# tyt0223/emqx

Measured on AMD Instinct MI355X. Metric: topics matched/sec (node) at 10M filters, 1/2/4/8 GPUs; % HBM roofline, higher is better.
Workload: dtype u32

## Files before the change

### emqx_amd/csrc/egm_bulk.cpp

```cpp
#include <stdio.h>
#include <stdlib.h>
#include <string.h>

#include <chrono>

#include <algorithm>
#include <string_view>
#include <thread>
#include <unordered_map>
#include <vector>

#include "egm_table.h"

namespace egm {

namespace {

template <class F>
void parallel_for(size_t n, unsigned nt, F fn) {
  if (n < nt) nt = (unsigned)n;
  if (nt <= 1) {
    fn((size_t)0, n, 0u);
    return;
  }
  std::vector<std::thread> th;
  for (unsigned t = 0; t < nt; ++t) {
    const size_t lo = n * t / nt, hi = n * (t + 1) / nt;
    th.emplace_back([=, &fn] { fn(lo, hi, t); });
  }
  for (auto& x : th) x.join();
}

template <class T>
void parallel_sort(std::vector<T>& v, unsigned nt) {
  const size_t n = v.size();
  if (nt <= 1 || n < (1u << 16)) {
    std::sort(v.begin(), v.end());
    return;
  }
  std::vector<size_t> b(nt + 1);
  for (unsigned t = 0; t <= nt; ++t) b[t] = n * t / nt;
  parallel_for(nt, nt, [&](size_t lo, size_t hi, unsigned) {
    for (size_t t = lo; t < hi; ++t) std::sort(v.begin() + b[t], v.begin() + b[t + 1]);
  });
  std::vector<T> tmp(n);
  std::vector<T>* src = &v;
  std::vector<T>* dst = &tmp;
  for (size_t w = 1; w < nt; w <<= 1) {
    std::vector<std::thread> th;
    for (size_t t = 0; t < nt; t += 2 * w) {
      const size_t a = b[t], m = b[std::min<size_t>(t + w, nt)], e = b[std::min<size_t>(t + 2 * w, nt)];
      th.emplace_back([=] { std::merge(src->begin() + a, src->begin() + m, src->begin() + m, src->begin() + e,
                                       dst->begin() + a); });
    }
    for (auto& x : th) x.join();
    std::swap(src, dst);
  }
  if (src != &v) v.swap(*src);
}

struct Item {
  uint64_t key;
  uint32_t li;
  uint32_t pad;
  bool operator<(const Item& o) const { return key != o.key ? key < o.key : li < o.li; }
};

template <class K>
std::vector<std::vector<uint32_t>> bin_by_range(size_t n, unsigned R, unsigned nt, K key) {
  std::vector<std::vector<std::vector<uint32_t>>> part(nt, std::vector<std::vector<uint32_t>>(R));
  parallel_for(n, nt, [&](size_t lo, size_t hi, unsigned t) {
    for (size_t i = lo; i < hi; ++i) {
      const uint32_t r = key(i);
      if (r < R) part[t][r].push_back((uint32_t)i);
    }
  });
  std::vector<std::vector<uint32_t>> out(R);
  parallel_for(R, nt, [&](size_t lo, size_t hi, unsigned) {
    for (size_t r = lo; r < hi; ++r)
      for (unsigned t = 0; t < nt; ++t) {
        out[r].insert(out[r].end(), part[t][r].begin(), part[t][r].end());
        std::vector<uint32_t>().swap(part[t][r]);
      }
  });
  return out;
}


}

unsigned build_threads() {
  const char* e = getenv("EGM_BUILD_THREADS");
  if (e && *e) return (unsigned)std::max(1, atoi(e));
  unsigned n = std::max(1u, std::thread::hardware_concurrency());
  if (FILE* f = fopen("/sys/fs/cgroup/cpu.max", "r")) {
    char q[64] = {0};
    unsigned long long period = 0;
    if (fscanf(f, "%63s %llu", q, &period) == 2 && strcmp(q, "max") != 0 && period) {
      const unsigned long long quota = strtoull(q, nullptr, 10);
      n = std::min<unsigned>(n, (unsigned)std::max<unsigned long long>(1, (quota + period - 1) / period));
    }
    fclose(f);
  }
  return std::min(n, 64u);
}

namespace {
struct Phase {
  bool on = getenv("EGM_BULK_TRACE") != nullptr;
  std::chrono::steady_clock::time_point t = std::chrono::steady_clock::now();
  void operator()(const char* what) {
    if (!on) return;
    const auto now = std::chrono::steady_clock::now();
    fprintf(stderr, "[egm bulk] %-22s %8.3f s\n", what, std::chrono::duration<double>(now - t).count());
    t = now;
  }
};
}

int HostTable::bulk_build(const uint8_t* blob, const uint32_t* off, uint32_t n, const uint32_t* ids, unsigned nt) {
  Phase phase;
  clear();
  if (nt == 0) nt = build_threads();
  std::vector<uint64_t> h(n);
  parallel_for(n, nt, [&](size_t lo, size_t hi, unsigned) {
    for (size_t i = lo; i < hi; ++i) h[i] = word_hash(blob + off[i], off[i + 1] - off[i]);
  });
  std::vector<uint8_t> dup(n, 0);
  {
    std::vector<Item> byh(n);
    parallel_for(n, nt, [&](size_t lo, size_t hi, unsigned) {
      for (size_t i = lo; i < hi; ++i) byh[i] = Item{h[i], (uint32_t)i, 0};
    });
    parallel_sort(byh, nt);
    parallel_for(n, nt, [&](size_t lo, size_t hi, unsigned) {
      for (size_t k = lo; k < hi; ++k) {
        if (k == 0 || byh[k - 1].key != byh[k].key) continue;
        const uint32_t i = byh[k].li, li = off[i + 1] - off[i];
        for (size_t j = k; j-- > 0 && byh[j].key == byh[k].key;) {
          const uint32_t p = byh[j].li;
          if (off[p + 1] - off[p] == li && memcmp(blob + off[p], blob + off[i], li) == 0) {
            dup[i] = 1;
            break;
          }
        }
      }
    });
  }
  phase("dedup");
  std::vector<uint32_t> uniq;
  uniq.reserve(n);
  for (uint32_t i = 0; i < n; ++i)
    if (!dup[i]) uniq.push_back(i);
  std::vector<uint8_t>().swap(dup);
  const uint32_t U = (uint32_t)uniq.size();
  foff_.assign((size_t)U + 1, 0);
  for (uint32_t r = 0; r < U; ++r) foff_[r + 1] = foff_[r] + (off[uniq[r] + 1] - off[uniq[r]]);
  fblob_.resize(foff_[U]);
  ffid_.resize(U);
  falive_.assign(U, 1);
  uint32_t max_fid = 0;
  parallel_for(U, nt, [&](size_t lo, size_t hi, unsigned) {
    for (size_t r = lo; r < hi; ++r) {
      const uint32_t i = uniq[r];
      memcpy(fblob_.data() + foff_[r], blob + off[i], off[i + 1] - off[i]);
      ffid_[r] = ids ? ids[i] : i;
    }
  });
  for (uint32_t r = 0; r < U; ++r) max_fid = std::max(max_fid, ffid_[r] + 1);
  n_filters_ = U;
  next_fid_ = U ? max_fid : 0;
  {
    std::vector<uint64_t> hb(U), hf(U);
    parallel_for(U, nt, [&](size_t lo, size_t hi, unsigned) {
      for (size_t r = lo; r < hi; ++r) {
        hb[r] = h[uniq[r]];
        hf[r] = mix64(ffid_[r]);
      }
    });
    std::vector<uint64_t>().swap(h);
    by_bytes_.bulk_build(hb, nt);
    by_fid_.bulk_build(hf, nt);
  }
  phase("filter store + maps");
  std::vector<uint64_t> tok_off((size_t)U + 1, 0);
  {
    std::vector<uint32_t> depth(U);
    parallel_for(U, nt, [&](size_t lo, size_t hi, unsigned) {
      for (size_t r = lo; r < hi; ++r) {
        const uint8_t* p = fblob_.data() + foff_[r];
        const uint64_t len = foff_[r + 1] - foff_[r];
        uint32_t d = 1;
        for (uint64_t k = 0; k < len; ++k) d += p[k] == '/';
        depth[r] = d;
      }
    });
    for (uint32_t r = 0; r < U; ++r) tok_off[r + 1] = tok_off[r] + depth[r];
  }
  std::vector<uint32_t> tok(tok_off[U]);
  {
    const unsigned T = (U < 4096) ? 1u : nt;
    std::vector<std::vector<std::string_view>> local(T);
    std::vector<std::vector<uint32_t>> to_global(T);
    parallel_for(U, T, [&](size_t lo, size_t hi, unsigned t) {
      std::unordered_map<std::string_view, uint32_t> seen;
      auto& lw = local[t];
      for (size_t r = lo; r < hi; ++r) {
        const uint8_t* p = fblob_.data() + foff_[r];
        const uint32_t len = (uint32_t)(foff_[r + 1] - foff_[r]);
        uint64_t o = tok_off[r];
        uint32_t s = 0;
        for (uint32_t i = 0; i <= len; ++i) {
          if (i < len && p[i] != '/') continue;
          const uint32_t wl = i - s;
          uint32_t v;
          if (wl == 1 && p[s] == '+') v = WID_PLUS;
          else if (wl == 1 && p[s] == '#') v = WID_HASH;
          else {
            std::string_view w((const char*)p + s, wl);
            auto it = seen.find(w);
            if (it == seen.end()) {
              it = seen.emplace(w, (uint32_t)lw.size()).first;
              lw.push_back(w);
            }
            v = it->second;
          }
          tok[o++] = v;
          s = i + 1;
        }
      }
    });
    size_t total = 0;
    for (auto& l : local) total += l.size();
    size_t cap = 64;
    while (cap < 2 * total) cap <<= 1;
    dict_rehash(cap);
    for (unsigned t = 0; t < T; ++t) {
      to_global[t].resize(local[t].size());
      for (size_t k = 0; k < local[t].size(); ++k)
        to_global[t][k] = dict_add((const uint8_t*)local[t][k].data(), (uint32_t)local[t][k].size());
    }
    parallel_for(U, T, [&](size_t lo, size_t hi, unsigned t) {
      const auto& g = to_global[t];
      for (uint64_t k = tok_off[lo]; k < tok_off[hi]; ++k)
        if (tok[k] < WID_MAX) tok[k] = g[tok[k]];
    });
  }
  phase("dictionary + tokens");
  std::vector<uint32_t> act(U), nxt;
  for (uint32_t r = 0; r < U; ++r) act[r] = r;
  std::vector<uint32_t> cur_node(U, 0);
  std::vector<NodeRec> nn(1, NodeRec{NONE, NONE, NONE, 0});
  std::vector<uint32_t> npar(1, NONE), nvia(1, NONE), nref(1, U), nhc(1, NONE);
  {
    const size_t bound = (size_t)tok_off[U] + 1;
    nn.reserve(bound + bound / 8 + 1024);
    for (auto* v : {&npar, &nvia, &nref, &nhc}) v->reserve(bound + bound / 8 + 1024);
  }
  struct Child {
    uint32_t token, first, count, start;
  };
  for (uint32_t level = 0; !act.empty(); ++level) {
    const size_t A = act.size();
    std::vector<size_t> cb{0};
    for (unsigned t = 1; t < nt; ++t) {
      size_t k = std::max(cb.back(), A * t / nt);
      while (k < A && k > 0 && cur_node[act[k]] == cur_node[act[k - 1]]) ++k;
      if (k > cb.back() && k < A) cb.push_back(k);
    }
    cb.push_back(A);
    const size_t C = cb.size() - 1;
    std::vector<std::vector<std::pair<uint64_t, uint32_t>>> citems(C);
    std::vector<std::vector<Child>> ckids(C);
    auto sort_chunk = [&](size_t c, unsigned inner) {
      auto& it = citems[c];
      auto& kids = ckids[c];
      it.resize(cb[c + 1] - cb[c]);
      for (size_t k = cb[c]; k < cb[c + 1]; ++k) {
        const uint32_t r = act[k];
        it[k - cb[c]] = {((uint64_t)tok[tok_off[r] + level] << 32) | r, cur_node[r]};
      }
      size_t a = 0;
      while (a < it.size()) {
        size_t e = a + 1;
        while (e < it.size() && it[e].second == it[a].second) ++e;
        if (e - a > 1) {
          if (inner > 1) {
            std::vector<std::pair<uint64_t, uint32_t>> run(it.begin() + a, it.begin() + e);
            parallel_sort(run, inner);
            std::copy(run.begin(), run.end(), it.begin() + a);
          } else {
            std::sort(it.begin() + a, it.begin() + e);
          }
        }
        const size_t k0 = kids.size();
        for (size_t k = a; k < e; ++k)
          if (k == a || (it[k].first >> 32) != (it[k - 1].first >> 32))
            kids.push_back(Child{(uint32_t)(it[k].first >> 32), (uint32_t)it[k].first, 0, (uint32_t)k});
        for (size_t g = k0; g < kids.size(); ++g)
          kids[g].count = (uint32_t)((g + 1 < kids.size() ? kids[g + 1].start : e) - kids[g].start);
        std::sort(kids.begin() + k0, kids.end(), [](const Child& x, const Child& y) { return x.first < y.first; });
        a = e;
      }
    };
    if (C == 1) sort_chunk(0, nt);
    else parallel_for(C, (unsigned)C, [&](size_t lo, size_t hi, unsigned) {
      for (size_t c = lo; c < hi; ++c) sort_chunk(c, 1);
    });
    std::vector<uint64_t> cbase(C + 1, nn.size());
    for (size_t c = 0; c < C; ++c) cbase[c + 1] = cbase[c] + ckids[c].size();
    if (cbase[C] >= (uint64_t)WID_MAX) return -1;
    const uint32_t N2 = (uint32_t)cbase[C];
    nn.resize(N2, NodeRec{NONE, NONE, NONE, 0});
    npar.resize(N2);
    nvia.resize(N2);
    nref.resize(N2);
    nhc.resize(N2, NONE);
    std::vector<uint64_t> nbase(C + 1, 0);
    std::vector<std::vector<uint32_t>> cnext(C);
    parallel_for(C, (unsigned)std::min<size_t>(C, nt), [&](size_t lo, size_t hi, unsigned) {
      for (size_t c = lo; c < hi; ++c) {
        const auto& it = citems[c];
        auto& out = cnext[c];
        out.reserve(it.size());
        for (size_t g = 0; g < ckids[c].size(); ++g) {
          const Child& k = ckids[c][g];
          const uint32_t node = (uint32_t)(cbase[c] + g), p = it[k.start].second;
          npar[node] = p;
          nvia[node] = k.token;
          nref[node] = k.count;
          if (k.token == WID_PLUS) nn[p].plus_child = node;
          else if (k.token == WID_HASH) nhc[p] = node;
          for (size_t q = k.start; q < (size_t)k.start + k.count; ++q) {
            const uint32_t r = (uint32_t)it[q].first;
            cur_node[r] = node;
            if (tok_off[r] + level + 1 == tok_off[r + 1]) {
              nn[node].term_fid = ffid_[r];
              if (k.token == WID_HASH) nn[p].hash_fid = ffid_[r];
            } else {
              out.push_back(r);
            }
          }
        }
        std::vector<std::pair<uint64_t, uint32_t>>().swap(citems[c]);
      }
    });
    for (size_t c = 0; c < C; ++c) nbase[c + 1] = nbase[c] + cnext[c].size();
    nxt.resize(nbase[C]);
    parallel_for(C, (unsigned)std::min<size_t>(C, nt), [&](size_t lo, size_t hi, unsigned) {
      for (size_t c = lo; c < hi; ++c) std::copy(cnext[c].begin(), cnext[c].end(), nxt.begin() + nbase[c]);
    });
    act.swap(nxt);
    phase("  level");
  }
  std::vector<uint32_t>().swap(cur_node);
  std::vector<uint32_t>().swap(tok);
  const uint32_t N = (uint32_t)nn.size();
  nodes.swap(nn);
  hash_child.swap(nhc);
  parent_.swap(npar);
  via_.swap(nvia);
  ref_.swap(nref);
  lit_count_.assign(N, 0);
  sig_.assign(N, 0);
  edge_slot_.assign(N, NONE);
  free_nodes_.clear();
  n_live_nodes_ = N;
  uint64_t n_lit = 0;
  for (uint32_t c = 1; c < N; ++c)
    if (via_[c] < WID_MAX) {
      ++lit_count_[parent_[c]];
      sig_[parent_[c]] |= sig_bit(via_[c]);
      ++n_lit;
    }
  parallel_for(N, nt, [&](size_t lo, size_t hi, unsigned) {
    for (size_t c = lo; c < hi; ++c) nodes[c].flags = own_flags((uint32_t)c);
  });
  const size_t room = N + N / 8 + 1024;
  for (auto* v : {&hash_child, &parent_, &via_, &ref_, &lit_count_, &sig_, &edge_slot_}) v->reserve(room);
  nodes.reserve(room);
  phase("node records");
  size_t nb = 16;
  while (nb * EDGE_BUCKET < (size_t)n_lit * EDGE_SPREAD) nb <<= 1;
  edges.assign(nb * EDGE_BUCKET, EdgeSlot{NONE, 0, 0, 0, NONE, NONE, NONE, 0});
  n_edges_ = n_lit;
  n_edge_tombs_ = 0;
  {
    const uint32_t m = (uint32_t)(nb - 1);
    const unsigned T = (n_lit < 65536) ? 1u : nt;
    std::vector<std::vector<uint32_t>> spill(T);
    auto bins = bin_by_range(N, T, nt, [&](size_t c) -> uint32_t {
      if (c == 0 || via_[c] >= WID_MAX) return T;
      return (uint32_t)((uint64_t)edge_bucket(parent_[c], via_[c], m) * T / nb);
    });
    parallel_for(T, T, [&](size_t lo, size_t hi, unsigned) {
      for (size_t t = lo; t < hi; ++t) {
        const uint64_t b1 = (uint64_t)nb * (t + 1) / T;
        for (uint32_t c : bins[t]) {
          const uint32_t b = edge_bucket(parent_[c], via_[c], m);
          bool placed = false;
          for (uint64_t bb = b; bb < b1 && !placed; ++bb)
            for (int k = 0; k < EDGE_BUCKET; ++k) {
              EdgeSlot& s = edges[bb * EDGE_BUCKET + k];
              if (s.parent != NONE) continue;
              const NodeRec& r = nodes[c];
              s = EdgeSlot{parent_[c], via_[c], c, r.flags, r.plus_child, r.hash_fid, r.term_fid, plus_flags(c)};
              edge_slot_[c] = (uint32_t)(bb * EDGE_BUCKET + k);
              placed = true;
              break;
            }
          if (!placed) spill[t].push_back(c);
        }
      }
    });
    for (auto& sp : spill)
      for (uint32_t c : sp) {
        uint32_t b = edge_bucket(parent_[c], via_[c], m);
        for (bool placed = false; !placed; b = (b + 1) & m)
          for (int k = 0; k < EDGE_BUCKET; ++k) {
            EdgeSlot& s = edges[(size_t)b * EDGE_BUCKET + k];
            if (s.parent != NONE) continue;
            const NodeRec& r = nodes[c];
            s = EdgeSlot{parent_[c], via_[c], c, r.flags, r.plus_child, r.hash_fid, r.term_fid, plus_flags(c)};
            edge_slot_[c] = (uint32_t)((size_t)b * EDGE_BUCKET + k);
            placed = true;
            break;
          }
      }
  }
  phase("edge table");
  dirty_.clear();
  dirty_.nodes_full = dirty_.edges_full = dirty_.dict_full = dirty_.words_full = true;
  return 0;
}

void IndexMap::bulk_build(const std::vector<uint64_t>& h, unsigned nt) {
  const size_t n = h.size();
  size_t cap = 16;
  while (cap < 4 * n) cap <<= 1;
  slots_.assign(cap, Slot{0, 0, 0});
  n_ = n;
  tombs_ = 0;
  const size_t m = cap - 1;
  const unsigned T = n < 65536 ? 1u : nt;
  std::vector<std::vector<uint32_t>> spill(T);
  auto bins = bin_by_range(n, T, nt, [&](size_t i) -> uint32_t { return (uint32_t)((h[i] & m) * T / cap); });
  parallel_for(T, T, [&](size_t lo, size_t hi, unsigned) {
    for (size_t t = lo; t < hi; ++t) {
      const size_t s1 = cap * (t + 1) / T;
      for (uint32_t i : bins[t]) {
        size_t j = h[i] & m;
        while (j < s1 && slots_[j].state == 1) ++j;
        if (j < s1) slots_[j] = Slot{h[i], i, 1};
        else spill[t].push_back(i);
      }
    }
  });
  for (auto& sp : spill)
    for (uint32_t i : sp) {
      size_t j = h[i] & m;
      while (slots_[j].state == 1) j = (j + 1) & m;
      slots_[j] = Slot{h[i], i, 1};
    }
}

}
```

### emqx_amd/csrc/egm_common.h

```cpp
#pragma once
#include <stdint.h>

#if defined(__HIPCC__)
#define EGM_HD __host__ __device__ __forceinline__
#else
#define EGM_HD inline
#endif

namespace egm {

constexpr uint32_t NONE = 0xFFFFFFFFu;
constexpr uint32_t TOMB = 0xFFFFFFFEu;

constexpr uint32_t WID_NONE = 0xFFFFFFFFu;
constexpr uint32_t WID_PLUS = 0xFFFFFFFDu;
constexpr uint32_t WID_HASH = 0xFFFFFFFCu;
constexpr uint32_t WID_MAX  = 0xFFFFFFF0u;

constexpr uint32_t F_LIT  = 1u;
constexpr uint32_t F_PLUS = 2u;
constexpr uint32_t F_HASH = 4u;
constexpr uint32_t F_TERM = 8u;

constexpr uint32_t F_BASIC = 0xFu;
constexpr uint32_t SIG_SHIFT = 4;
constexpr uint32_t SIG_BITS = 28;

constexpr uint8_t TF_WILDCARD = 1;
constexpr uint8_t TF_DOLLAR   = 2;
constexpr uint8_t TF_HEAVY    = 4;
constexpr uint8_t TF_ERROR    = 8;
constexpr uint8_t TF_SKIP     = 16;

#ifndef EGM_EDGE_BUCKET
#define EGM_EDGE_BUCKET 2
#endif
constexpr int EDGE_BUCKET = EGM_EDGE_BUCKET;
static_assert(EDGE_BUCKET == 2 || EDGE_BUCKET == 4, "a bucket is one or two 64-B lines");
#ifndef EGM_EDGE_SPREAD
#define EGM_EDGE_SPREAD 2
#endif
constexpr uint32_t EDGE_SPREAD = EGM_EDGE_SPREAD;

struct NodeRec {
  uint32_t plus_child;
  uint32_t hash_fid;
  uint32_t term_fid;
  uint32_t flags;
};

struct EdgeSlot {
  uint32_t parent;
  uint32_t wid;
  uint32_t child;
  uint32_t child_flags;
  uint32_t child_plus;
  uint32_t child_hash;
  uint32_t child_term;
  uint32_t child_pflags;
};

struct DictSlot {
  uint64_t hash;
  uint32_t wid;
  uint32_t len;
  uint8_t inl[16];
};

static_assert(sizeof(NodeRec) == 16, "NodeRec");
static_assert(sizeof(EdgeSlot) == 32, "EdgeSlot");
static_assert(sizeof(DictSlot) == 32, "DictSlot");

constexpr uint64_t FNV_BASIS = 0xcbf29ce484222325ull;
constexpr uint64_t FNV_PRIME = 0x100000001b3ull;

EGM_HD uint64_t mix64(uint64_t x) {
  x ^= x >> 33;
  x *= 0xff51afd7ed558ccdull;
  x ^= x >> 33;
  x *= 0xc4ceb9fe1a85ec53ull;
  x ^= x >> 33;
  return x;
}

EGM_HD uint64_t hash_chunk(uint64_t h, uint32_t c) { return (h ^ c) * FNV_PRIME; }

EGM_HD uint64_t word_hash_finish(uint64_t h, uint32_t len) {
  return mix64(h ^ ((uint64_t)len << 56));
}

EGM_HD uint64_t word_hash(const uint8_t* p, uint32_t len) {
  uint64_t h = FNV_BASIS;
  uint32_t i = 0;
  for (; i + 4 <= len; i += 4)
    h = hash_chunk(h, (uint32_t)p[i] | ((uint32_t)p[i + 1] << 8) | ((uint32_t)p[i + 2] << 16) |
                          ((uint32_t)p[i + 3] << 24));
  if (i < len) {
    uint32_t c = 0;
    for (uint32_t k = 0; i + k < len; ++k) c |= (uint32_t)p[i + k] << (8 * k);
    h = hash_chunk(h, c);
  }
  return word_hash_finish(h, len);
}

EGM_HD uint32_t sig_index(uint32_t wid) {
#ifdef EGM_SIG_HASH32
  const uint32_t h = wid * 0x9E3779B1u;
#else
  const uint32_t h = (uint32_t)(mix64(0x9E3779B97F4A7C15ull ^ wid) >> 32);
#endif
  return (uint32_t)(((uint64_t)h * SIG_BITS) >> 32);
}

EGM_HD uint32_t sig_bit(uint32_t wid) {
  return 1u << (SIG_SHIFT + sig_index(wid));
}

EGM_HD uint32_t edge_bucket(uint32_t parent, uint32_t wid, uint32_t mask) {
#ifdef EGM_EDGE_HASH32
  uint32_t h = (parent * 0x9E3779B1u) ^ wid;
  h ^= h >> 16;
  h *= 0x85EBCA6Bu;
  h ^= h >> 13;
  return h & mask;
#else
  return (uint32_t)(mix64(((uint64_t)parent << 32) | wid) & mask);
#endif
}

EGM_HD uint32_t prefix_key_len(const uint8_t* p, uint32_t len) {
  uint32_t slashes = 0;
  for (uint32_t i = 0; i < len; ++i)
    if (p[i] == '/' && ++slashes == 2) return i;
  return len;
}

EGM_HD uint32_t prefix_vpart(const uint8_t* p, uint32_t len, uint32_t n_vparts) {
  return (uint32_t)(word_hash(p, prefix_key_len(p, len)) % n_vparts);
}

EGM_HD bool prefix_replicated(const uint8_t* p, uint32_t len) {
  uint32_t ws = 0, level = 0;
  for (uint32_t i = 0; i <= len && level < 2; ++i) {
    if (i < len && p[i] != '/') continue;
    if (i - ws == 1 && (p[ws] == '+' || p[ws] == '#')) return true;
    ws = i + 1;
    ++level;
  }
  return false;
}

EGM_HD uint32_t filter_shard(const uint8_t* p, uint32_t len, uint32_t n_shards) {
  return (uint32_t)(word_hash(p, len) % n_shards);
}

}
```

### emqx_amd/csrc/egm_table.cpp

```cpp
#include "egm_table.h"

#include <string.h>

#include <algorithm>

namespace egm {

static size_t pow2_at_least(size_t n) {
  size_t c = 16;
  while (c < n) c <<= 1;
  return c;
}

void IndexMap::reserve(size_t n) {
  if (slots_.size() < 2 * n) grow(2 * n);
}

void IndexMap::grow(size_t want) {
  std::vector<Slot> old;
  old.swap(slots_);
  slots_.assign(pow2_at_least(want), Slot{0, 0, 0});
  n_ = 0;
  tombs_ = 0;
  for (const Slot& s : old)
    if (s.state == 1) insert(s.h, s.v);
}

template <class Eq>
uint32_t IndexMap::find(uint64_t h, Eq eq) const {
  if (slots_.empty()) return NONE;
  size_t m = slots_.size() - 1, i = h & m;
  for (;;) {
    const Slot& s = slots_[i];
    if (s.state == 0) return NONE;
    if (s.state == 1 && s.h == h && eq(s.v)) return s.v;
    i = (i + 1) & m;
  }
}

void IndexMap::insert(uint64_t h, uint32_t v) {
  if ((n_ + tombs_ + 1) * 2 > slots_.size()) grow(std::max<size_t>(32, (n_ + 1) * 4));
  size_t m = slots_.size() - 1, i = h & m;
  while (slots_[i].state == 1) i = (i + 1) & m;
  if (slots_[i].state == 2) --tombs_;
  slots_[i] = Slot{h, v, 1};
  ++n_;
}

template <class Eq>
bool IndexMap::erase(uint64_t h, Eq eq) {
  if (slots_.empty()) return false;
  size_t m = slots_.size() - 1, i = h & m;
  for (;;) {
    Slot& s = slots_[i];
    if (s.state == 0) return false;
    if (s.state == 1 && s.h == h && eq(s.v)) {
      s.state = 2;
      --n_;
      ++tombs_;
      return true;
    }
    i = (i + 1) & m;
  }
}

static void append_or_full(std::vector<uint32_t>& v, bool& full, const std::vector<uint32_t>& o) {
  if (full) return;
  v.insert(v.end(), o.begin(), o.end());
}

void DirtyLog::merge(const DirtyLog& o) {
  nodes_full |= o.nodes_full;
  edges_full |= o.edges_full;
  dict_full |= o.dict_full;
  words_full |= o.words_full;
  append_or_full(nodes, nodes_full, o.nodes);
  append_or_full(edges, edges_full, o.edges);
  append_or_full(dict, dict_full, o.dict);
  if (nodes_full) std::vector<uint32_t>().swap(nodes);
  if (edges_full) std::vector<uint32_t>().swap(edges);
  if (dict_full) std::vector<uint32_t>().swap(dict);
}

void DirtyLog::clear() {
  std::vector<uint32_t>().swap(nodes);
  std::vector<uint32_t>().swap(edges);
  std::vector<uint32_t>().swap(dict);
  nodes_full = edges_full = dict_full = words_full = false;
}

void HostTable::mark_node(uint32_t n) {
  if (dirty_.nodes_full) return;
  dirty_.nodes.push_back(n);
  if (dirty_.nodes.size() > nodes.size() / 4 + 4096) {
    dirty_.nodes_full = true;
    std::vector<uint32_t>().swap(dirty_.nodes);
  }
}

void HostTable::mark_edge(uint32_t s) {
  if (dirty_.edges_full) return;
  dirty_.edges.push_back(s);
  if (dirty_.edges.size() > edges.size() / 4 + 4096) {
    dirty_.edges_full = true;
    std::vector<uint32_t>().swap(dirty_.edges);
  }
}

DirtyLog HostTable::take_dirty() {
  DirtyLog d;
  std::swap(d, dirty_);
  return d;
}

HostTable::HostTable() { clear(); }

void HostTable::clear() {
  dirty_.clear();
  dirty_.nodes_full = dirty_.edges_full = dirty_.dict_full = dirty_.words_full = true;
  nodes.clear();
  hash_child.clear();
  parent_.clear();
  via_.clear();
  ref_.clear();
  lit_count_.clear();
  sig_.clear();
  edge_slot_.clear();
  free_nodes_.clear();
  n_live_nodes_ = 0;
  edges.assign(16 * EDGE_BUCKET, EdgeSlot{NONE, 0, 0, 0, NONE, NONE, NONE, 0});
  n_edges_ = n_edge_tombs_ = 0;
  dict.assign(64, DictSlot{0, NONE, 0, {0}});
  dict_blob.clear();
  dict_off.assign(1, 0);
  n_dict_used_ = 0;
  fblob_.clear();
  foff_.assign(1, 0);
  ffid_.clear();
  falive_.clear();
  by_bytes_ = IndexMap();
  by_fid_ = IndexMap();
  n_filters_ = 0;
  next_fid_ = 0;
  new_node(NONE, NONE);
}

uint32_t HostTable::new_node(uint32_t parent, uint32_t via) {
  uint32_t n;
  if (!free_nodes_.empty()) {
    n = free_nodes_.back();
    free_nodes_.pop_back();
  } else {
    n = (uint32_t)nodes.size();
    nodes.push_back({});
    hash_child.push_back(NONE);
    parent_.push_back(NONE);
    via_.push_back(NONE);
    ref_.push_back(0);
    lit_count_.push_back(0);
    sig_.push_back(0);
    edge_slot_.push_back(NONE);
  }
  nodes[n] = NodeRec{NONE, NONE, NONE, 0};
  hash_child[n] = NONE;
  parent_[n] = parent;
  via_[n] = via;
  ref_[n] = 0;
  lit_count_[n] = 0;
  sig_[n] = 0;
  edge_slot_[n] = NONE;
  ++n_live_nodes_;
  mark_node(n);
  return n;
}

void HostTable::free_node(uint32_t n) {
  nodes[n] = NodeRec{NONE, NONE, NONE, 0};
  hash_child[n] = NONE;
  parent_[n] = NONE;
  via_[n] = NONE;
  edge_slot_[n] = NONE;
  free_nodes_.push_back(n);
  --n_live_nodes_;
  mark_node(n);
}

uint32_t HostTable::own_flags(uint32_t n) const {
  const NodeRec& r = nodes[n];
  return (lit_count_[n] ? F_LIT | sig_[n] : 0u) | (r.plus_child != NONE ? F_PLUS : 0u) |
         (r.hash_fid != NONE ? F_HASH : 0u) | (r.term_fid != NONE ? F_TERM : 0u);
}

void HostTable::update_flags(uint32_t n) {
  NodeRec& r = nodes[n];
  r.flags = own_flags(n);
  mark_node(n);
  const uint32_t par = parent_[n];
  if (par != NONE && via_[n] == WID_PLUS && parent_[par] != NONE && via_[par] < WID_MAX) {
    mark_edge(edge_slot_[par]);
    edges[edge_slot_[par]].child_pflags = r.flags;
  }
  if (par == NONE || via_[n] >= WID_MAX) return;
  mark_edge(edge_slot_[n]);
  EdgeSlot& s = edges[edge_slot_[n]];
  s.child_flags = r.flags;
  s.child_plus = r.plus_child;
  s.child_hash = r.hash_fid;
  s.child_term = r.term_fid;
  s.child_pflags = plus_flags(n);
}

uint32_t HostTable::plus_flags(uint32_t n) const {
  return nodes[n].plus_child != NONE ? nodes[nodes[n].plus_child].flags : 0u;
}

uint32_t HostTable::dict_find(const uint8_t* p, uint32_t len) const {
  uint64_t h = word_hash(p, len);
  uint32_t m = dict_mask(), i = (uint32_t)(h & m);
  for (;;) {
    const DictSlot& s = dict[i];
    if (s.wid == NONE) return NONE;
    if (s.hash == h && s.len == len && memcmp(dict_blob.data() + dict_off[s.wid], p, len) == 0)
      return s.wid;
    i = (i + 1) & m;
  }
}

void HostTable::dict_rehash(size_t cap) {
  std::vector<DictSlot> old;
  old.swap(dict);
  dict.assign(cap, DictSlot{0, NONE, 0, {0}});
  dirty_.dict_full = true;
  std::vector<uint32_t>().swap(dirty_.dict);
  uint32_t m = (uint32_t)cap - 1;
  for (const DictSlot& s : old) {
    if (s.wid == NONE) continue;
    uint32_t i = (uint32_t)(s.hash & m);
    while (dict[i].wid != NONE) i = (i + 1) & m;
    dict[i] = s;
  }
}

uint32_t HostTable::dict_add(const uint8_t* p, uint32_t len) {
  uint32_t w = dict_find(p, len);
  if (w != NONE) return w;
  if ((size_t)(n_dict_used_ + 1) * 2 > dict.size()) dict_rehash(dict.size() * 2);
  w = (uint32_t)dict_off.size() - 1;
  dict_blob.insert(dict_blob.end(), p, p + len);
  dict_off.push_back(dict_blob.size());
  uint64_t h = word_hash(p, len);
  uint32_t m = dict_mask(), i = (uint32_t)(h & m);
  while (dict[i].wid != NONE) i = (i + 1) & m;
  DictSlot s{h, w, len, {0}};
  memcpy(s.inl, p, len < 16 ? len : 16);
  dict[i] = s;
  if (!dirty_.dict_full) dirty_.dict.push_back(i);
  ++n_dict_used_;
  return w;
}

uint32_t HostTable::edge_find(uint32_t parent, uint32_t wid) const {
  uint32_t m = edge_mask(), b = edge_bucket(parent, wid, m);
  for (;;) {
    bool has_empty = false;
    for (int k = 0; k < EDGE_BUCKET; ++k) {
      const EdgeSlot& s = edges[(size_t)b * EDGE_BUCKET + k];
      if (s.parent == parent && s.wid == wid) return (uint32_t)(b * EDGE_BUCKET + k);
      if (s.parent == NONE) has_empty = true;
    }
    if (has_empty) return NONE;
    b = (b + 1) & m;
  }
}

uint32_t HostTable::edge_insert(uint32_t parent, uint32_t wid, uint32_t child, uint32_t cflags) {
  size_t nb = edges.size() / EDGE_BUCKET;
  if ((n_edges_ + n_edge_tombs_ + 1) * EDGE_SPREAD > nb * EDGE_BUCKET) {
    size_t want = nb;
    while ((n_edges_ + 1) * EDGE_SPREAD > want * EDGE_BUCKET / 2) want *= 2;
    edge_rehash(want);
  }
  uint32_t m = edge_mask(), b = edge_bucket(parent, wid, m);
  for (;;) {
    for (int k = 0; k < EDGE_BUCKET; ++k) {
      EdgeSlot& s = edges[(size_t)b * EDGE_BUCKET + k];
      if (s.parent == NONE || s.parent == TOMB) {
        if (s.parent == TOMB) --n_edge_tombs_;
        const NodeRec& r = nodes[child];
        s = EdgeSlot{parent, wid, child, cflags, r.plus_child, r.hash_fid, r.term_fid, plus_flags(child)};
        ++n_edges_;
        mark_edge((uint32_t)(b * EDGE_BUCKET + k));
        return (uint32_t)(b * EDGE_BUCKET + k);
      }
    }
    b = (b + 1) & m;
  }
}

void HostTable::edge_rehash(size_t n_buckets) {
  std::vector<EdgeSlot> old;
  old.swap(edges);
  edges.assign(n_buckets * EDGE_BUCKET, EdgeSlot{NONE, 0, 0, 0, NONE, NONE, NONE, 0});
  n_edges_ = n_edge_tombs_ = 0;
  dirty_.edges_full = true;
  std::vector<uint32_t>().swap(dirty_.edges);
  for (const EdgeSlot& s : old) {
    if (s.parent == NONE || s.parent == TOMB) continue;
    uint32_t slot = edge_insert(s.parent, s.wid, s.child, s.child_flags);
    edge_slot_[s.child] = slot;
  }
}

uint32_t HostTable::find_local(const uint8_t* p, uint32_t len, uint64_t h) const {
  return by_bytes_.find(h, [&](uint32_t li) {
    uint64_t a = foff_[li], b = foff_[li + 1];
    return falive_[li] && b - a == len && memcmp(fblob_.data() + a, p, len) == 0;
  });
}

uint32_t HostTable::lookup(const uint8_t* p, uint32_t len) const {
  uint32_t li = find_local(p, len, word_hash(p, len));
  return li == NONE ? NONE : ffid_[li];
}

bool HostTable::id_in_use(uint32_t fid) const {
  return by_fid_.find(mix64(fid), [&](uint32_t x) { return falive_[x] && ffid_[x] == fid; }) != NONE;
}

const uint8_t* HostTable::filter_bytes(uint32_t fid, uint32_t* len) const {
  uint32_t li = by_fid_.find(mix64(fid), [&](uint32_t x) { return falive_[x] && ffid_[x] == fid; });
  if (li == NONE) return nullptr;
  *len = (uint32_t)(foff_[li + 1] - foff_[li]);
  return fblob_.data() + foff_[li];
}

int HostTable::insert(const uint8_t* p, uint32_t len, uint32_t fid, uint32_t* out_fid) {
  uint64_t h = word_hash(p, len);
  uint32_t li = find_local(p, len, h);
  if (li != NONE) {
    if (out_fid) *out_fid = ffid_[li];
    return 1;
  }
  if (fid == NONE) fid = next_fid_;
  if (fid >= WID_MAX) return -1;
  if (by_fid_.find(mix64(fid), [&](uint32_t x) { return falive_[x] && ffid_[x] == fid; }) != NONE)
    return -2;
  if (fid >= next_fid_) next_fid_ = fid + 1;

  uint32_t cur = 0;
  uint32_t start = 0;
  bool last_hash = false;
  for (uint32_t i = 0; i <= len; ++i) {
    if (i < len && p[i] != '/') continue;
    const uint8_t* w = p + start;
    uint32_t wl = i - start;
    start = i + 1;
    uint32_t c;
    last_hash = false;
    if (wl == 1 && w[0] == '+') {
      c = nodes[cur].plus_child;
      if (c == NONE) {
        c = new_node(cur, WID_PLUS);
        nodes[cur].plus_child = c;
        update_flags(c);
        update_flags(cur);
      }
    } else if (wl == 1 && w[0] == '#') {
      c = hash_child[cur];
      if (c == NONE) {
        c = new_node(cur, WID_HASH);
        hash_child[cur] = c;
        mark_node(cur);
      }
      last_hash = true;
    } else {
      uint32_t wid = dict_add(w, wl);
      uint32_t s = edge_find(cur, wid);
      if (s == NONE) {
        c = new_node(cur, wid);
        s = edge_insert(cur, wid, c, 0);
        edge_slot_[c] = s;
        ++lit_count_[cur];
        sig_[cur] |= sig_bit(wid);
        update_flags(cur);
      } else {
        c = edges[s].child;
      }
    }
    ++ref_[c];
    cur = c;
  }
  ++ref_[0];
  nodes[cur].term_fid = fid;
  update_flags(cur);
  if (last_hash) {
    uint32_t par = parent_[cur];
    nodes[par].hash_fid = fid;
    update_flags(par);
  }

  uint32_t nli = (uint32_t)ffid_.size();
  fblob_.insert(fblob_.end(), p, p + len);
  foff_.push_back(fblob_.size());
  ffid_.push_back(fid);
  falive_.push_back(1);
  by_bytes_.insert(h, nli);
  by_fid_.insert(mix64(fid), nli);
  ++n_filters_;
  if (out_fid) *out_fid = fid;
  return 0;
}

int HostTable::remove(const uint8_t* p, uint32_t len) {
  uint64_t h = word_hash(p, len);
  uint32_t li = find_local(p, len, h);
  if (li == NONE) return 1;
  uint32_t fid = ffid_[li];

  std::vector<uint32_t> path;
  uint32_t cur = 0, start = 0;
  for (uint32_t i = 0; i <= len; ++i) {
    if (i < len && p[i] != '/') continue;
    const uint8_t* w = p + start;
    uint32_t wl = i - start;
    start = i + 1;
    if (wl == 1 && w[0] == '+') cur = nodes[cur].plus_child;
    else if (wl == 1 && w[0] == '#') cur = hash_child[cur];
    else cur = edges[edge_find(cur, dict_find(w, wl))].child;
    path.push_back(cur);
  }
  uint32_t term = path.back();
  nodes[term].term_fid = NONE;
  update_flags(term);
  if (via_[term] == WID_HASH) {
    nodes[parent_[term]].hash_fid = NONE;
    update_flags(parent_[term]);
  }
  for (size_t k = path.size(); k-- > 0;) {
    uint32_t n = path[k];
    if (--ref_[n] != 0) continue;
    uint32_t par = parent_[n];
    if (via_[n] == WID_PLUS) {
      nodes[par].plus_child = NONE;
    } else if (via_[n] == WID_HASH) {
      hash_child[par] = NONE;
    } else {
      edges[edge_slot_[n]].parent = TOMB;
      mark_edge(edge_slot_[n]);
      --n_edges_;
      ++n_edge_tombs_;
      --lit_count_[par];
    }
    free_node(n);
    update_flags(par);
  }
  --ref_[0];

  by_bytes_.erase(h, [&](uint32_t x) { return x == li; });
  by_fid_.erase(mix64(fid), [&](uint32_t x) { return x == li; });
  falive_[li] = 0;
  --n_filters_;
  return 0;
}

void HostTable::relayout() {
  dirty_.nodes_full = dirty_.edges_full = true;
  std::vector<uint32_t>().swap(dirty_.nodes);
  std::vector<uint32_t>().swap(dirty_.edges);
  const uint32_t N = (uint32_t)nodes.size();
  std::vector<uint32_t> cnt(N + 1, 0);
  for (uint32_t n = 1; n < N; ++n)
    if (parent_[n] != NONE) ++cnt[parent_[n] + 1];
  for (uint32_t i = 0; i < N; ++i) cnt[i + 1] += cnt[i];
  std::vector<uint32_t> kids(cnt[N]);
  {
    std::vector<uint32_t> pos(cnt.begin(), cnt.end() - 1);
    for (uint32_t n = 1; n < N; ++n)
      if (parent_[n] != NONE) kids[pos[parent_[n]]++] = n;
  }
  std::vector<uint32_t> order;
  order.reserve(n_live_nodes_);
  std::vector<uint32_t> newid(N, NONE);
  order.push_back(0);
  newid[0] = 0;
  for (size_t qi = 0; qi < order.size(); ++qi) {
    uint32_t n = order[qi];
    for (uint32_t k = cnt[n]; k < cnt[n + 1]; ++k) {
      uint32_t c = kids[k];
      newid[c] = (uint32_t)order.size();
      order.push_back(c);
    }
  }
  const uint32_t L = (uint32_t)order.size();
  std::vector<NodeRec> nn(L);
  std::vector<uint32_t> nhc(L), npar(L), nvia(L), nref(L), nlit(L);
  for (uint32_t i = 0; i < L; ++i) {
    uint32_t o = order[i];
    NodeRec r = nodes[o];
    if (r.plus_child != NONE) r.plus_child = newid[r.plus_child];
    nn[i] = r;
    nhc[i] = hash_child[o] == NONE ? NONE : newid[hash_child[o]];
    npar[i] = parent_[o] == NONE ? NONE : newid[parent_[o]];
    nvia[i] = via_[o];
    nref[i] = ref_[o];
    nlit[i] = lit_count_[o];
  }
  std::vector<uint32_t>().swap(sig_);
  sig_.assign(L, 0);
  nodes.swap(nn);
  hash_child.swap(nhc);
  parent_.swap(npar);
  via_.swap(nvia);
  ref_.swap(nref);
  lit_count_.swap(nlit);
  edge_slot_.assign(L, NONE);
  free_nodes_.clear();
  n_live_nodes_ = L;
  const size_t room = L + L / 8 + 1024;
  for (auto* v : {&hash_child, &parent_, &via_, &ref_, &lit_count_, &sig_, &edge_slot_}) v->reserve(room);
  nodes.reserve(room);

  size_t nb = 16;
  while (nb * EDGE_BUCKET < (size_t)n_edges_ * EDGE_SPREAD) nb <<= 1;
  std::vector<EdgeSlot> old;
  old.swap(edges);
  edges.assign(nb * EDGE_BUCKET, EdgeSlot{NONE, 0, 0, 0, NONE, NONE, NONE, 0});
  n_edges_ = n_edge_tombs_ = 0;
  std::vector<EdgeSlot> live;
  live.reserve(old.size());
  for (const EdgeSlot& s : old)
    if (s.parent != NONE && s.parent != TOMB) live.push_back(s);
  for (EdgeSlot& s : live) {
    s.parent = newid[s.parent];
    s.child = newid[s.child];
  }
  std::sort(live.begin(), live.end(), [](const EdgeSlot& a, const EdgeSlot& b) { return a.child < b.child; });
  for (const EdgeSlot& s : live) sig_[s.parent] |= sig_bit(s.wid);
  for (uint32_t n = 0; n < L; ++n) nodes[n].flags = own_flags(n);
  for (const EdgeSlot& s : live)
    edge_slot_[s.child] = edge_insert(s.parent, s.wid, s.child, nodes[s.child].flags);
}

}
```

Measured before the change: 1.220 billion.

## Renumber trie nodes so plus-wildcard children are packed contiguously

Both bulk build and relayout now give nodes reached through a '+' edge the lowest IDs, placed just after the root. All other nodes follow in their previous order. The intent is better cache and HBM locality for the wildcard walk, since plus children are visited for every topic. The renumbering is parallel in bulk build, with the node arrays permuted and the child and parent pointers remapped. The cost is an extra permutation pass at build time, and the BFS locality between siblings is lost for plus nodes.

After: 1.261 billion, median of 6. 1.03x the previous value.

```diff
diff --git a/emqx_amd/csrc/egm_bulk.cpp b/emqx_amd/csrc/egm_bulk.cpp
--- a/emqx_amd/csrc/egm_bulk.cpp
+++ b/emqx_amd/csrc/egm_bulk.cpp
@@ -7,6 +7,7 @@
 #include <algorithm>
 #include <string_view>
 #include <thread>
+#include <type_traits>
 #include <unordered_map>
 #include <vector>
 
@@ -356,6 +357,46 @@
   std::vector<uint32_t>().swap(cur_node);
   std::vector<uint32_t>().swap(tok);
   const uint32_t N = (uint32_t)nn.size();
+  if (N > 1) {
+    std::vector<uint32_t> pbase(nt + 1, 0);
+    parallel_for(N, nt, [&](size_t lo, size_t hi, unsigned t) {
+      uint32_t k = 0;
+      for (size_t c = lo; c < hi; ++c) k += nvia[c] == WID_PLUS;
+      pbase[t + 1] = k;
+    });
+    for (unsigned t = 0; t < nt; ++t) pbase[t + 1] += pbase[t];
+    const uint32_t P = pbase[nt];
+    if (P) {
+      std::vector<uint32_t> newid(N);
+      parallel_for(N, nt, [&](size_t lo, size_t hi, unsigned t) {
+        uint32_t np = 1 + pbase[t], no = P + 1 + (lo ? (uint32_t)lo - 1 - pbase[t] : 0u);
+        for (size_t c = lo; c < hi; ++c) newid[c] = c == 0 ? 0u : nvia[c] == WID_PLUS ? np++ : no++;
+      });
+      const size_t room = N + N / 8 + 1024;
+      auto remap = [&](uint32_t x) { return x == NONE ? NONE : newid[x]; };
+      auto permute = [&](auto& v, auto& out, auto fix) {
+        out.reserve(room);
+        out.resize(N);
+        parallel_for(N, nt, [&](size_t lo, size_t hi, unsigned) {
+          for (size_t c = lo; c < hi; ++c) out[newid[c]] = fix(v[c]);
+        });
+        v.swap(out);
+      };
+      {
+        std::vector<NodeRec> spare;
+        permute(nn, spare, [&](NodeRec r) {
+          r.plus_child = remap(r.plus_child);
+          return r;
+        });
+      }
+      std::vector<uint32_t> spare;
+      permute(nhc, spare, remap);
+      permute(npar, spare, remap);
+      permute(nvia, spare, [](uint32_t x) { return x; });
+      permute(nref, spare, [](uint32_t x) { return x; });
+    }
+  }
+  phase("node layout");
   nodes.swap(nn);
   hash_child.swap(nhc);
   parent_.swap(npar);
diff --git a/emqx_amd/csrc/egm_common.h b/emqx_amd/csrc/egm_common.h
--- a/emqx_amd/csrc/egm_common.h
+++ b/emqx_amd/csrc/egm_common.h
@@ -41,6 +41,8 @@
 #define EGM_EDGE_SPREAD 2
 #endif
 constexpr uint32_t EDGE_SPREAD = EGM_EDGE_SPREAD;
+
+constexpr uint32_t NODE_LAYOUT_VERSION = 2;
 
 struct NodeRec {
   uint32_t plus_child;
diff --git a/emqx_amd/csrc/egm_table.cpp b/emqx_amd/csrc/egm_table.cpp
--- a/emqx_amd/csrc/egm_table.cpp
+++ b/emqx_amd/csrc/egm_table.cpp
@@ -478,20 +478,31 @@
     for (uint32_t n = 1; n < N; ++n)
       if (parent_[n] != NONE) kids[pos[parent_[n]]++] = n;
   }
-  std::vector<uint32_t> order;
-  order.reserve(n_live_nodes_);
+  std::vector<uint32_t> bfs;
+  bfs.reserve(n_live_nodes_);
+  bfs.push_back(0);
+  uint32_t P = 0;
+  for (size_t qi = 0; qi < bfs.size(); ++qi) {
+    uint32_t n = bfs[qi];
+    for (uint32_t k = cnt[n]; k < cnt[n + 1]; ++k) {
+      bfs.push_back(kids[k]);
+      P += via_[kids[k]] == WID_PLUS;
+    }
+  }
+  const uint32_t L = (uint32_t)bfs.size();
+  std::vector<uint32_t> order(L);
   std::vector<uint32_t> newid(N, NONE);
-  order.push_back(0);
-  newid[0] = 0;
-  for (size_t qi = 0; qi < order.size(); ++qi) {
-    uint32_t n = order[qi];
-    for (uint32_t k = cnt[n]; k < cnt[n + 1]; ++k) {
-      uint32_t c = kids[k];
-      newid[c] = (uint32_t)order.size();
-      order.push_back(c);
-    }
-  }
-  const uint32_t L = (uint32_t)order.size();
+  {
+    uint32_t np = 1, no = P + 1;
+    for (uint32_t i = 1; i < L; ++i) {
+      const uint32_t o = bfs[i], id = via_[o] == WID_PLUS ? np++ : no++;
+      order[id] = o;
+      newid[o] = id;
+    }
+    order[0] = 0;
+    newid[0] = 0;
+  }
+  std::vector<uint32_t>().swap(bfs);
   std::vector<NodeRec> nn(L);
   std::vector<uint32_t> nhc(L), npar(L), nvia(L), nref(L), nlit(L);
   for (uint32_t i = 0; i < L; ++i) {
```
